# pavelacamposp/direct_data_driven_mpc

Measured on AMD Instinct MI355X. Metric: QP solves/sec (batched), four-tank robust DD-MPC L=30 N=400, higher is better.
Workload: dtype f64

## Files before the change

### direct_data_driven_mpc_amd/csrc/ddmpc_cold2.hpp

```cpp
#pragma once
#include "ddmpc_kernels.hpp"

namespace ddmpc {

template <int NT, int W>
struct TileMap2 {
  struct Tab { int wave[NT]; int base[NT]; int maxs; };
  static constexpr Tab make() {
    Tab t{};
    int load[W] = {};
    t.wave[0] = 0; t.base[0] = 0; load[0] = NT;
    for (int d = 1; d < NT; ++d) {
      int w = (W > 1) ? 1 : 0;
      for (int i = w + 1; i < W; ++i) if (load[i] < load[w]) w = i;
      t.wave[d] = w;
      t.base[d] = load[w];
      load[w] += NT - d;
    }
    t.maxs = 0;
    for (int i = 0; i < W; ++i) if (load[i] > t.maxs) t.maxs = load[i];
    return t;
  }
  static constexpr Tab tab = make();
  static constexpr int MAXS = tab.maxs;
  static constexpr int wave(int I, int J) { return tab.wave[I - J]; }
  static constexpr int slot(int I, int J) { return tab.base[I - J] + J; }
  static constexpr bool has_row(int w, int J) {
    for (int K = 0; K < J; ++K) if (wave(J, K) == w) return true;
    return false;
  }
  static constexpr bool has_col(int w, int J) {
    for (int I = J + 1; I < NT; ++I) if (wave(I, J) == w) return true;
    return false;
  }
};

template <int NT, int W, int WAVE>
struct WaveTiles2 {
  struct Tab { int I[NT * (NT + 1) / 2]; int J[NT * (NT + 1) / 2]; int n; };
  static constexpr Tab make() {
    Tab t{};
    t.n = 0;
    for (int J = 0; J < NT; ++J)
      for (int I = J; I < NT; ++I)
        if (TileMap2<NT, W>::wave(I, J) == WAVE) { t.I[t.n] = I; t.J[t.n] = J; ++t.n; }
    return t;
  }
  static constexpr Tab tab = make();
};

template <int CTRL>
__device__ __forceinline__ double dpp_mov_f64(double v) {
  const int lo = __builtin_amdgcn_update_dpp(0, __double2loint(v), CTRL, 0xf, 0xf, false);
  const int hi = __builtin_amdgcn_update_dpp(0, __double2hiint(v), CTRL, 0xf, 0xf, false);
  return __hiloint2double(hi, lo);
}
__device__ __forceinline__ double row16_total(double v) {
  v += dpp_mov_f64<0x128>(v);
  v += dpp_mov_f64<0x124>(v);
  v += dpp_mov_f64<0x122>(v);
  v += dpp_mov_f64<0x121>(v);
  return v;
}

__device__ __forceinline__ d2 permlane16_swap_f64(double a, double b) {
  const auto lo = __builtin_amdgcn_permlane16_swap((unsigned)__double2loint(a), (unsigned)__double2loint(b), false, false);
  const auto hi = __builtin_amdgcn_permlane16_swap((unsigned)__double2hiint(a), (unsigned)__double2hiint(b), false, false);
  return d2{__hiloint2double((int)hi[0], (int)lo[0]), __hiloint2double((int)hi[1], (int)lo[1])};
}

__device__ __forceinline__ double rsq_n2(double x) {
  const double y0 = __builtin_amdgcn_rsq(x);
  const double e = fma(-x * y0, y0, 1.0);
  return fma(0.5 * y0, e, y0);
}

__device__ __forceinline__ double rows4_total(double v) {
  const d2 s1 = permlane16_swap_f64(v, v);
  v = s1[0] + s1[1];
  const auto lo2 = __builtin_amdgcn_permlane32_swap((unsigned)__double2loint(v), (unsigned)__double2loint(v), false, false);
  const auto hi2 = __builtin_amdgcn_permlane32_swap((unsigned)__double2hiint(v), (unsigned)__double2hiint(v), false, false);
  return __hiloint2double((int)hi2[0], (int)lo2[0]) + __hiloint2double((int)hi2[1], (int)lo2[1]);
}

__device__ __forceinline__ double wave_max(double v) {
  v = fmax(v, dpp_mov_f64<0x128>(v));
  v = fmax(v, dpp_mov_f64<0x124>(v));
  v = fmax(v, dpp_mov_f64<0x122>(v));
  v = fmax(v, dpp_mov_f64<0x121>(v));
  const d2 s1 = permlane16_swap_f64(v, v);
  v = fmax(s1[0], s1[1]);
  const auto lo2 = __builtin_amdgcn_permlane32_swap((unsigned)__double2loint(v), (unsigned)__double2loint(v), false, false);
  const auto hi2 = __builtin_amdgcn_permlane32_swap((unsigned)__double2hiint(v), (unsigned)__double2hiint(v), false, false);
  return fmax(__hiloint2double((int)hi2[0], (int)lo2[0]), __hiloint2double((int)hi2[1], (int)lo2[1]));
}

template <int NT, int W>
struct Lds2 {
  static constexpr int RP = 16 * NT;
  static constexpr int dvec = 0;
  static constexpr int tvec = dvec + RP;
  static constexpr int beta = tvec + RP;
  static constexpr int cd0 = beta + RP;
  static constexpr int cd1 = cd0 + RP;
  static constexpr int ct0 = cd1 + RP;
  static constexpr int ckk = ct0 + RP;
  static constexpr int PART_LEN = 2 * 16 * W;
  static constexpr int part = ckk + (RP + 1) / 2;
  static constexpr int RED_LEN = 34;
  static constexpr int red = part + PART_LEN;
  static constexpr int ints = red + RED_LEN;
  static constexpr int INTS_LEN = (RP + 8 + 1) / 2;
  static constexpr int pt2 = (ints + INTS_LEN + 2) & ~1;
  static constexpr int PT2_LEN = 32 * 4;
  static constexpr int LRS = 36;
  static constexpr int lt16 = pt2 + PT2_LEN;
  static constexpr int LT_LEN = 16 * LRS;
  static constexpr int pastw = lt16;
  static constexpr int PASTW_CAP = LT_LEN / 2;
  static constexpr int cpp = lt16 + PASTW_CAP;
  static constexpr int RSB = RP + 4;
  static constexpr int pb = lt16 + LT_LEN;
  static constexpr int PB_LEN = 16 * RSB;
  static constexpr int ctab = pb + PB_LEN;
  static constexpr int CTAB_LEN = 4 * RP;
  static constexpr bool DST_ALIAS = RP >= 128;
  static constexpr int dst = ctab + CTAB_LEN;
  static constexpr int DST_LEN = (W > 1 && !DST_ALIAS) ? 256 : 0;
  static constexpr int dst_lo = DST_ALIAS ? dvec : dst;
  static constexpr int dst_hi = DST_ALIAS ? beta : dst + 128;
  static constexpr int xs = dst + DST_LEN;
  static constexpr int SCR = pt2;
  static constexpr int SCR_LEN = dst - pt2;
  __host__ __device__ static constexpr int total(int xs_len) { return (xs + xs_len + 1) & ~1; }

  static_assert(W >= 1 && W <= 8, "red[] keeps 8 per-wave slots per quantity; part[] is sized by W");
  static_assert(24 + W <= 32 && RED_LEN >= 33, "red[24 + w] and red[32] (output stage) must stay inside red[]");
  static_assert(pt2 >= ints + INTS_LEN && (pt2 & 1) == 0, "act[RP] + flags[8] end before the in-tile panel; 16-byte aligned");
  static_assert(cpp + (RP + 1) / 2 <= lt16 + LT_LEN, "prologue staging (past window + its index table) must fit inside lt16");
  static_assert(NT * 256 <= PB_LEN, "back substitution keeps the NT inverse diagonal tiles M_J in the panel buffer");
  static_assert(16 * (RP / 4) <= CTAB_LEN, "one 4x4 lag block per time step of the window");
  static_assert((xs & 1) == 0 && (lt16 & 1) == 0 && (pb & 1) == 0, "16-byte alignment of the regions accessed with b128");
};

template <int NT, int W>
struct Lds2Limits {
  static constexpr int max_past = Lds2<NT, W>::PASTW_CAP;
  static constexpr int scratch = Lds2<NT, W>::SCR_LEN;
};

template <int NT, int W, int WAVE, bool REF, bool CVX>
__device__ __forceinline__ void wave_body2(const KParams& P, double* __restrict__ sm,
                                           const double* __restrict__ up, const double* __restrict__ yp,
                                           double* __restrict__ u_opt, double* __restrict__ cost_out,
                                           int* __restrict__ status_out, int* __restrict__ iters_out,
                                           double* __restrict__ beta_ws, signed char* __restrict__ act_ws,
                                           unsigned long long* __restrict__ stamps, double* __restrict__ lfac,
                                           double* __restrict__ lfacT, int* __restrict__ refine_flag,
                                           int* __restrict__ refine_count, const double* __restrict__ gpre,
                                           const double* __restrict__ ud_b, const double* __restrict__ yd_b) {
  using TM = TileMap2<NT, W>;
  using WT = WaveTiles2<NT, W, WAVE>;
  using LD = Lds2<NT, W>;
  constexpr int RP = 16 * NT;
  constexpr int NTHR = 64 * W;
  constexpr int LRS = LD::LRS, RSB = LD::RSB;
  int nstamp = 1;
  auto stamp = [&]() __attribute__((always_inline)) {
    if (stamps != nullptr && WAVE == 0) {
      const unsigned long long t = __builtin_amdgcn_s_memtime();
      if (threadIdx.x == 0 && nstamp < 7) stamps[nstamp] = t;
      ++nstamp;
    }
  };
  double* xs = sm + LD::xs;
  double* dvec = sm + LD::dvec;
  double* tvec = sm + LD::tvec;
  double* beta = sm + LD::beta;
  double* part = sm + LD::part;
  double* red = sm + LD::red;
  double* ctab = sm + LD::ctab;
  double* PT2 = sm + LD::pt2;
  double* LT = sm + LD::lt16;
  double* PB = sm + LD::pb;
  int* act = reinterpret_cast<int*>(sm + LD::ints);
  int* flags = act + RP;

  int tid0 = threadIdx.x;
  asm volatile("" : "+v"(tid0));
  const int r = P.r, rE = P.rE, nch = P.nch;
  const int NS = rE >> 2;
  const int IR = rE >> 4;
  const int rr = rE & 15;

  constexpr int NHELP = (W > 1) ? W - 1 : 1;
  constexpr int DFIRST = 3;
  constexpr int NDSLOT = (W > 1 && NT > DFIRST) ? (NT - DFIRST + NHELP - 1) / NHELP : 1;
  auto downer = [](int J) constexpr { return 1 + (J - DFIRST) % NHELP; };
  auto dslot = [](int J) constexpr { return (J - DFIRST) / NHELP; };
  static_assert(8 * (TM::MAXS + (W > 1 ? NDSLOT : 0)) + 40 <= 512 / DDMPC_MIN_WAVES(NT, W),
                "the accumulator tiles of the busiest wave must leave a working set of 40 VGPRs at the occupancy of __launch_bounds__");
  d4 acc[TM::MAXS];
  d4 dlt[NDSLOT];
  double* DSTlo = sm + LD::dst_lo;
  double* DSThi = sm + LD::dst_hi;

  constexpr int NE = (RP + NTHR - 1) / NTHR;
  double* cD0 = sm + LD::cd0;
  double* cD1 = sm + LD::cd1;
  double* cT = sm + LD::ct0;
  int* cK = reinterpret_cast<int*>(sm + LD::ckk);
  {
    const int* cP = reinterpret_cast<const int*>(sm + LD::cpp);
    const double* pastw = sm + LD::pastw;
    static_for<NE>([&](auto e) __attribute__((always_inline)) {
      const int rho = tid0 + e * NTHR;
      if (rho < RP) {
        const int pidx = cP[rho];
        if (pidx >= 0) cT[rho] = pastw[pidx];
        act[rho] = 0;
      }
    });
  }
  if (tid0 < 8) flags[tid0] = 0;

  int iter = 0;
  int status = 0;
  int nupd = 0;
  bool ctab_ok = false;
  int tid = tid0;
  double kmax = 0.0;
  long long tphF = 0, tphB = 0, tphT = 0, tphA = 0, tphU = 0;
  const bool timing = (stamps != nullptr) && (WAVE == 0);
  auto now = [&]() __attribute__((always_inline)) -> long long { return timing ? (long long)__builtin_amdgcn_s_memtime() : 0; };
  for (;;) {
    ++iter;
    asm volatile("" : "+v"(tid));
    int r_it = P.r, rE_it = P.rE;
    asm volatile("" : "+s"(r_it), "+s"(rE_it));
    const int r = r_it, rE = rE_it;
    const int NS = rE >> 2, IR = rE >> 4, rr = rE & 15;
    const int lane = tid & 63;
    const int l15 = lane & 15, l4 = lane >> 4, l3 = lane & 3, lo = l15 >> 2;
    int ix_x = lane & 31, ix_lt = l4 * LRS + l15, ix_pw = l4 * 4 + l3;
    if constexpr (WAVE == 0) asm volatile("" : "+v"(ix_x), "+v"(ix_lt), "+v"(ix_pw));
    static_for<NE>([&](auto e) __attribute__((always_inline)) {
      const int rho = tid + e * NTHR;
      if (rho < RP) {
        const int s_act = act[rho];
        dvec[rho] = s_act ? cD1[rho] : cD0[rho];
        tvec[rho] = cT[rho] + s_act * P.bound;
        beta[rho] = 0.0;
      }
    });
    if (tid == 0) flags[1] = 0;
    __syncthreads();
    stamp();

    bool f0_done = false;
    static_for<NDSLOT>([&](auto S) __attribute__((always_inline)) { dlt[S] = d4{0.0, 0.0, 0.0, 0.0}; });
    bool dst_valid = false;
    auto fix_tile = [&](auto II, auto JJ, const d4& raw, const double dd) __attribute__((always_inline)) -> d4 {
      constexpr int I = II, J = JJ;
      const int gc = 16 * I + l15;
      d4 v = -raw;
      if constexpr (I == J) {
        const bool live = gc < r;
        const int dj = l15 - l4;
        static_for<4>([&](auto j) __attribute__((always_inline)) {
          const bool hit = live && (dj == 4 * j);
          if (hit) { asm volatile(""); kmax = fmax(kmax, raw[j()]); v[j()] -= P.lam * dd; }
        });
      }
      if (16 * I + 15 >= r) {
        double tg[4];
        static_for<4>([&](auto j) __attribute__((always_inline)) { tg[j()] = tvec[16 * J + l4 + 4 * j]; });
        double tc = 0.0;
        if constexpr (I == J) tc = tvec[gc];
        static_for<4>([&](auto j) __attribute__((always_inline)) {
          const int gr = 16 * J + l4 + 4 * j;
          if (gr >= r || gc >= r) v[j()] = 0.0;
          if (I == J && gr == gc && gr >= r && gr < rE) v[j()] = -1.0;
          if (gc == rE && gr < r) v[j()] = -tg[j()];
          if (I == J && gr == rE && gc < r) v[j()] = -tc;
        });
      }
      if (P.dense_w) {
        const double* dm = P.dmat + (long long)(16 * J + l4) * RP + 16 * I + l15;
        static_for<4>([&](auto j) __attribute__((always_inline)) { v[j()] -= P.lam * dm[4 * j() * RP]; });
      }
      return v;
    };
    auto substep = [&](d4& Ad, d4& Et, d4& Mt, auto QQ, auto&& pend) __attribute__((always_inline)) {
      constexpr int q = QQ;
      constexpr int c0 = 4 * q;
#define DDMPC_HOOK(h) do { pend(std::integral_constant<int, h>{}); } while (0)
      const double* Pr = PT2 + 4 * ix_x;
      const double* Pd = PT2 + c0 * 4;
      const double p00 = -Pd[0];
      const double p10 = -Pd[4], p11 = -Pd[5];
      const double p20 = -Pd[8], p21 = -Pd[9], p22 = -Pd[10];
      const double p30 = -Pd[12], p31 = -Pd[13], p32 = -Pd[14], p33 = -Pd[15];
      const double r0 = Pr[0], r1 = Pr[1], r2 = Pr[2], r3 = Pr[3];
      double m0 = 0.0, m1 = 0.0, m2 = 0.0;
      if constexpr (q == 3) {
        m0 = LT[ix_lt + 16]; m1 = LT[ix_lt + 4 * LRS + 16]; m2 = LT[ix_lt + 8 * LRS + 16];
      }
      DDMPC_HOOK(0);
      const double i0 = rsq_n2(p00);
      DDMPC_HOOK(1);
      const double l10 = p10 * i0, l20 = p20 * i0, l30 = p30 * i0;
      const double i1 = rsq_n2(p11 - l10 * l10);
      DDMPC_HOOK(2);
      const double l21 = (p21 - l20 * l10) * i1, l31 = (p31 - l30 * l10) * i1;
      const double i2 = rsq_n2(p22 - l20 * l20 - l21 * l21);
      DDMPC_HOOK(3);
      const double l32 = (p32 - l30 * l20 - l31 * l21) * i2;
      const double i3 = rsq_n2(p33 - l30 * l30 - l31 * l31 - l32 * l32);
      DDMPC_HOOK(4);
      const double x0 = -r0 * i0;
      const double x1 = -(r1 + x0 * l10) * i1;
      DDMPC_HOOK(5);
      const double x2 = -(r2 + x0 * l20 + x1 * l21) * i2;
      const double x3 = -(r3 + x0 * l30 + x1 * l31 + x2 * l32) * i3;
      DDMPC_HOOK(6);
      const d2 s01a = permlane16_swap_f64(x0, x1), s23a = permlane16_swap_f64(x2, x3);
      const bool lowhalf = lane < 32;
      const double opA = lowhalf ? s01a[0] : s23a[0];
      const double opE = lowhalf ? s01a[1] : s23a[1];
      LT[ix_lt + c0 * LRS] = opA;
      LT[ix_lt + c0 * LRS + 16] = opE;
      if constexpr (q == 3) Mt = d4{m0, m1, m2, opE};
      DDMPC_HOOK(7);
      if constexpr (q < 3) {
        Ad = __builtin_amdgcn_mfma_f64_16x16x4f64(opA, opA, Ad, 0, 0, 0);
        Et = __builtin_amdgcn_mfma_f64_16x16x4f64(opE, opA, Et, 0, 0, 0);
      }
      DDMPC_HOOK(8);
      DDMPC_HOOK(9);
      DDMPC_HOOK(10);
      DDMPC_HOOK(11);
      if constexpr (q < 3) {
        if (lo == q + 1) {
          static_for<4>([&](auto j) __attribute__((always_inline)) {
            PT2[ix_pw + 16 * j] = Ad[j()];
            PT2[ix_pw + 16 * j + 64] = Et[j()];
          });
        }
      }
      __builtin_amdgcn_fence(__ATOMIC_ACQ_REL, "wavefront");
#undef DDMPC_HOOK
    };
    auto no_pend = [](auto) __attribute__((always_inline)) {};
    auto factor_begin = [&](const d4& Ad, d4& Et) __attribute__((always_inline)) {
      int lz = lane;
      asm volatile("" : "+v"(lz));
      static_for<4>([&](auto j) __attribute__((always_inline)) { Et[j()] = ((lz >> 4) + 4 * j() == (lz & 15)) ? -1.0 : 0.0; });
      if (lo == 0) {
        static_for<4>([&](auto j) __attribute__((always_inline)) {
          PT2[ix_pw + 16 * j] = Ad[j()];
          PT2[ix_pw + 16 * j + 64] = Et[j()];
        });
      }
      __builtin_amdgcn_fence(__ATOMIC_ACQ_REL, "wavefront");
    };
    auto factor_end = [&](auto JT, int nq) __attribute__((always_inline)) {
      constexpr int Jt = JT;
      constexpr int SD = TM::slot(Jt, Jt);
      __builtin_amdgcn_fence(__ATOMIC_ACQ_REL, "wavefront");
      if (nq < 4) {
        static_for<4>([&](auto j) __attribute__((always_inline)) {
          const int k = l4 + 4 * j();
          const double mv = LT[k * LRS + 16 + l15];
          acc[SD][j()] = (k < 4 * nq) ? mv : 0.0;
        });
      }
      if (Jt == IR) {
        if (lane < 4 * nq) tvec[16 * Jt + lane] = LT[lane * LRS + rr];
      }
      if (lfac != nullptr) {
        static_for<4>([&](auto e) __attribute__((always_inline)) {
          const int idx = lane + 64 * e(), xr = idx >> 4, kc = idx & 15;
          double v = (kc <= xr && kc < 4 * nq) ? LT[kc * LRS + xr] : 0.0;
          if (xr == kc && kc >= 4 * nq) v = 1.0;
          lfac[(Jt * (Jt + 1) / 2 + Jt) * 256 + idx] = v;
          lfacT[(Jt * (Jt + 1) / 2 + Jt) * 256 + kc * 16 + xr] = v;
        });
      }
    };
    if (gpre != nullptr) {
      static_for<WT::tab.n>([&](auto K) __attribute__((always_inline)) {
        constexpr int I = WT::tab.I[K], J = WT::tab.J[K];
        acc[TM::slot(I, J)] = *reinterpret_cast<const d4*>(gpre + (I * (I + 1) / 2 + J) * 256 + 4 * lane);
      });
      stamp();
      stamp();
    } else if (P.gram_dense) {
      static_for<TM::MAXS>([&](auto S) __attribute__((always_inline)) { acc[S] = d4{0.0, 0.0, 0.0, 0.0}; });
      const int c = P.c;
      const int cfull = c & ~3;
      const double* xp = xs + l4 * nch + l15;
      for (int i0 = 0; i0 < cfull; i0 += 4) {
        double op[NT];
        static_for<NT>([&](auto I) __attribute__((always_inline)) { op[I] = xp[16 * I]; });
        xp += 4 * nch;
        static_for<WT::tab.n>([&](auto K) __attribute__((always_inline)) {
          constexpr int I = WT::tab.I[K], J = WT::tab.J[K];
          acc[TM::slot(I, J)] = __builtin_amdgcn_mfma_f64_16x16x4f64(op[J], op[I], acc[TM::slot(I, J)], 0, 0, 0);
        });
      }
      if (cfull < c) {
        const bool kok = (cfull + l4) < c;
        double op[NT];
        static_for<NT>([&](auto I) __attribute__((always_inline)) { const double v = xp[16 * I]; op[I] = kok ? v : 0.0; });
        static_for<WT::tab.n>([&](auto K) __attribute__((always_inline)) {
          constexpr int I = WT::tab.I[K], J = WT::tab.J[K];
          acc[TM::slot(I, J)] = __builtin_amdgcn_mfma_f64_16x16x4f64(op[J], op[I], acc[TM::slot(I, J)], 0, 0, 0);
        });
      }
      stamp();
      stamp();
    } else {
      const int nsub = (nch == 2) ? 2 : 1;
      const int Ln = (nch == 2) ? (P.Ln + 1) >> 1 : P.Ln;
      auto csub = [&](int sub) __attribute__((always_inline)) { return (nch == 2) ? ((P.c + 1 - sub) >> 1) : P.c; };
      {
        constexpr int TS = (W >= 4) ? 4 : W;
        constexpr int GS = W / TS;
        constexpr int MAXG = (NT + GS - 1) / GS;
        static_assert(TS * GS == W, "waves = time slices x group slices");
        static_assert(TS * GS * MAXG * 64 <= LD::PT2_LEN + LD::LT_LEN + LD::PB_LEN, "partial lag blocks fit between pt2 and ctab");
        const int ngroups = (Ln + 3) >> 2;
        const int kq = lane >> 4, blk = (lane >> 2) & 3, ij = lane & 3;
        double* PP = sm + LD::pt2;
        constexpr int tsl = WAVE % TS, gsl = WAVE / TS;
        const bool need_lag = CVX ? !ctab_ok : (iter == 1);
        if (need_lag) {
          double cacc[MAXG];
          static_for<MAXG>([&](auto gi) __attribute__((always_inline)) { cacc[gi()] = 0.0; });
#pragma nounroll
          for (int sub = 0; sub < nsub; ++sub) {
          const int c = csub(sub);
          const double* xb = xs + 2 * sub;
          const int cfull = c & ~3;
          const int nks = cfull >> 2;
          const int kw = (nks + TS - 1) / TS;
          const int ks0 = tsl * kw;
          const int ks1 = (ks0 + kw) < nks ? (ks0 + kw) : nks;
          const double* pB = xb + 4 * (kq + 4 * ks0) + ij;
          const double* pA = xb + 4 * (kq + blk + 4 * ks0) + ij + 16 * (gsl * MAXG);
          auto ld = [&](double (&bv)[4], double (&av)[MAXG + 3]) __attribute__((always_inline)) {
            static_for<4>([&](auto u) __attribute__((always_inline)) { bv[u()] = pB[16 * u]; });
            static_for<MAXG + 3>([&](auto q) __attribute__((always_inline)) { av[q()] = pA[16 * q]; });
            pA += 64; pB += 64;
          };
          auto mm = [&](const double (&bv)[4], const double (&av)[MAXG + 3]) __attribute__((always_inline)) {
            static_for<4>([&](auto u) __attribute__((always_inline)) {
              static_for<MAXG>([&](auto gi) __attribute__((always_inline)) {
                cacc[gi()] = __builtin_amdgcn_mfma_f64_4x4x4f64(av[gi() + u()], bv[u()], cacc[gi()], 0, 0, 0);
              });
            });
          };
          const int nk = ks1 > ks0 ? ks1 - ks0 : 0;
          const int ntrip = nk >> 2;
          double bv0[4], av0[MAXG + 3];
#pragma nounroll
          for (int it = 0; it < ntrip; ++it) {
            ld(bv0, av0);
            mm(bv0, av0);
          }
          for (int k = 4 * ntrip; k < nk; ++k) {
            const double bv = pB[0];
            static_for<MAXG>([&](auto gi) __attribute__((always_inline)) {
              cacc[gi()] = __builtin_amdgcn_mfma_f64_4x4x4f64(pA[16 * gi], bv, cacc[gi()], 0, 0, 0);
            });
            pA += 16; pB += 16;
          }
          if (tsl == TS - 1 && cfull < c) {
            const bool kok = (cfull + kq) < c;
            const double bv = kok ? pB[0] : 0.0;
            static_for<MAXG>([&](auto gi) __attribute__((always_inline)) {
              const double a1 = pA[16 * gi];
              cacc[gi()] = __builtin_amdgcn_mfma_f64_4x4x4f64(kok ? a1 : 0.0, bv, cacc[gi()], 0, 0, 0);
            });
          }
          }
          static_for<MAXG>([&](auto gi) __attribute__((always_inline)) {
            PP[((tsl * GS + gsl) * MAXG + gi()) * 64 + lane] = cacc[gi()];
          });
        }
        __syncthreads();
        if (need_lag) {
          for (int e = tid; e < GS * MAXG * 64; e += NTHR) {
            const int g = e >> 6, ln = e & 63;
            double sacc = 0.0;
            static_for<TS>([&](auto t) __attribute__((always_inline)) { sacc += PP[(t() * GS * MAXG + g) * 64 + ln]; });
            const int d = 4 * g + ((ln >> 2) & 3);
            if (g < ngroups && d < Ln) ctab[d * 16 + (ln >> 4) * 4 + (ln & 3)] = sacc;
          }
        }
      }
      __syncthreads();
      ctab_ok = true;
      stamp();
      static_for<TM::MAXS>([&](auto S) __attribute__((always_inline)) { acc[S] = d4{0.0, 0.0, 0.0, 0.0}; });
      {
#pragma nounroll
        for (int d = 0; d < NT; ++d) {
          bool mine = false;
          static_for<NT>([&](auto DD) __attribute__((always_inline)) {
            if constexpr (TM::tab.wave[DD] == WAVE) mine = mine || (d == DD);
          });
          if (!mine) continue;
          auto base = [&](int j) __attribute__((always_inline)) -> double {
            int del = 4 * d + lo - j;
            const bool neg = del < 0;
            del = neg ? -del : del;
            del = del >= Ln ? Ln - 1 : del;
            const int pa = neg ? l4 : l3, pb = neg ? l3 : l4;
            const int nl = neg ? lo : j;
            double t = ctab[del * 16 + pa * 4 + pb];
#pragma nounroll
            for (int sub = 0; sub < nsub; ++sub) {
              const int c = csub(sub);
              const double* qa0 = xs + 2 * sub + 4 * del + pa;
              const double* qa1 = qa0 + 4 * c;
              const double* qb0 = xs + 2 * sub + pb;
              const double* qb1 = qb0 + 4 * c;
              const double e0 = qa1[0] * qb1[0] - qa0[0] * qb0[0];
              const double e1 = qa1[4] * qb1[4] - qa0[4] * qb0[4];
              const double e2 = qa1[8] * qb1[8] - qa0[8] * qb0[8];
              t += (0 < nl) ? e0 : 0.0;
              t += (1 < nl) ? e1 : 0.0;
              t += (2 < nl) ? e2 : 0.0;
            }
            return t;
          };
          const d4 v = d4{base(0), base(1), base(2), base(3)};
          static_for<NT>([&](auto DD) __attribute__((always_inline)) {
            if constexpr (TM::tab.wave[DD] == WAVE) { if (d == DD) acc[TM::slot(DD, 0)] = v; }
          });
        }
      }
      static_for<NT>([&](auto DD) __attribute__((always_inline)) {
        constexpr int d = DD;
        if constexpr (TM::tab.wave[d] == WAVE && d + 1 < NT) {
          const double* pb = xs + 4 * l4 + l15;
          const double* pa = pb + 16 * d;
          auto walk = [&](auto NSUB) __attribute__((always_inline)) {
            constexpr bool two = NSUB() == 2;
            const double* pa2 = pa + 4 * csub(0);
            const double* pb2 = pb + 4 * csub(0);
            const double* pa4 = pa + 2 + 4 * csub(1);
            const double* pb4 = pb + 2 + 4 * csub(1);
            double n_a1 = pa[0], n_b1 = pb[0], n_a2 = pa2[0], n_b2 = pb2[0];
            double n_a3 = 0.0, n_b3 = 0.0, n_a4 = 0.0, n_b4 = 0.0;
            if constexpr (two) { n_a3 = pa[2]; n_b3 = pb[2]; n_a4 = pa4[0]; n_b4 = pb4[0]; }
            static_for<NT - d - 1>([&](auto T) __attribute__((always_inline)) {
              const double a1 = n_a1, b1 = n_b1, a2 = n_a2, b2 = n_b2, a3 = n_a3, b3 = n_b3, a4 = n_a4, b4 = n_b4;
              if constexpr (T() + 1 < NT - d - 1) {
                constexpr int o = 16 * (T() + 1);
                n_a1 = pa[o]; n_b1 = pb[o]; n_a2 = pa2[o]; n_b2 = pb2[o];
                if constexpr (two) { n_a3 = pa[o + 2]; n_b3 = pb[o + 2]; n_a4 = pa4[o]; n_b4 = pb4[o]; }
              }
              d4 v = __builtin_amdgcn_mfma_f64_16x16x4f64(-b1, a1, acc[TM::slot(d + T, T)], 0, 0, 0);
              if constexpr (two) {
                v = __builtin_amdgcn_mfma_f64_16x16x4f64(-b3, a3, v, 0, 0, 0);
                v = __builtin_amdgcn_mfma_f64_16x16x4f64(b4, a4, v, 0, 0, 0);
              }
              acc[TM::slot(d + T + 1, T + 1)] = __builtin_amdgcn_mfma_f64_16x16x4f64(b2, a2, v, 0, 0, 0);
            });
          };
          if (nsub == 2) walk(std::integral_constant<int, 2>{});
          else walk(std::integral_constant<int, 1>{});
        }
      });
      if constexpr (WAVE == 0 && W > 1) {
        if (rE >= 16) {
          constexpr int S0 = TM::slot(0, 0);
          d4 Ad = fix_tile(std::integral_constant<int, 0>{}, std::integral_constant<int, 0>{}, acc[S0], dvec[l15]);
          d4 Et;
          factor_begin(Ad, Et);
          static_for<4>([&](auto q) __attribute__((always_inline)) { substep(Ad, Et, acc[S0], q, no_pend); });
          factor_end(std::integral_constant<int, 0>{}, 4);
          f0_done = true;
        }
      }
      stamp();
    }

    const long long tfx0 = now();
    double dgv[NT];
    static_for<WT::tab.n>([&](auto K) __attribute__((always_inline)) {
      constexpr int I = WT::tab.I[K], J = WT::tab.J[K];
      if constexpr (I == J) dgv[J] = dvec[16 * J + l15];
    });
    static_for<WT::tab.n>([&](auto K) __attribute__((always_inline)) {
      constexpr int I = WT::tab.I[K], J = WT::tab.J[K];
      constexpr int S = TM::slot(I, J);
      if (!(I == 0 && J == 0 && f0_done))
        acc[S] = fix_tile(std::integral_constant<int, I>{}, std::integral_constant<int, J>{}, acc[S], I == J ? dgv[J] : 0.0);
    });
    const long long tfx1 = now();
    if constexpr (W > 1 && WAVE >= 1 && WAVE <= 3) {
      if (stamps != nullptr) {
        const unsigned long long th = __builtin_amdgcn_s_memtime();
        if (lane == 0) stamps[6 + WAVE] = th << 32;
      }
    }
    __syncthreads();
    if constexpr (!CVX) {
      if (timing && threadIdx.x == 0) {
        const long long tfx2 = now();
        stamps[10] = (unsigned long long)(tfx1 - tfx0) << 32;
        stamps[11] = (unsigned long long)(tfx2 - tfx1) << 32;
      }
    }

    {
      const int nq0 = NS < 4 ? NS : 4;
      const long long t0 = now();
      if constexpr (WAVE == 0) {
        if (!f0_done) {
          d4 Ad = acc[TM::slot(0, 0)];
          d4 Et;
          factor_begin(Ad, Et);
          static_for<4>([&](auto q) __attribute__((always_inline)) { if (q() < nq0) substep(Ad, Et, acc[TM::slot(0, 0)], q, no_pend); });
          factor_end(std::integral_constant<int, 0>{}, nq0);
        }
      }
      const long long t1 = now();
      __syncthreads();
      tphF += t1 - t0; tphB += now() - t1;
    }
    static_for<NT>([&](auto JB) __attribute__((always_inline)) {
      constexpr int Jb = JB;
      const int nqc = (NS - 4 * Jb) < 4 ? (NS - 4 * Jb) : 4;
      if (nqc > 0) {
        const bool more = 16 * (Jb + 1) < rE + 1;
        const int nqn = (NS - 4 * (Jb + 1)) < 4 ? (NS - 4 * (Jb + 1)) : 4;
        const long long t0 = now();
        if constexpr (WAVE == 0 && W > 1 && Jb >= 1 && Jb + DFIRST - 1 < NT) {
          if (dst_valid) {
            constexpr int SDn = TM::slot(Jb + DFIRST - 1, Jb + DFIRST - 1);
            acc[SDn][0] += DSTlo[lane]; acc[SDn][1] += DSTlo[64 + lane];
            acc[SDn][2] += DSThi[lane]; acc[SDn][3] += DSThi[64 + lane];
          }
        }
        dst_valid = false;
        double am[4];
        static_for<4>([&](auto ks) __attribute__((always_inline)) { am[ks()] = -LT[l15 * LRS + 16 + 4 * ks() + l4]; });
        auto trsm_tile = [&](auto II) __attribute__((always_inline)) {
          constexpr int I = II;
          if (16 * I < rE + 1) {
            constexpr int S = TM::slot(I, Jb);
            const d4 T = acc[S];
            d4 dd = d4{0.0, 0.0, 0.0, 0.0};
            dd = __builtin_amdgcn_mfma_f64_16x16x4f64(am[0], T[0], dd, 0, 0, 0);
            dd = __builtin_amdgcn_mfma_f64_16x16x4f64(am[1], T[1], dd, 0, 0, 0);
            dd = __builtin_amdgcn_mfma_f64_16x16x4f64(am[2], T[2], dd, 0, 0, 0);
            dd = __builtin_amdgcn_mfma_f64_16x16x4f64(am[3], T[3], dd, 0, 0, 0);
            acc[S] = dd;
            static_for<4>([&](auto j) __attribute__((always_inline)) { PB[(l4 + 4 * j) * RSB + 16 * I + l15] = dd[j()]; });
          }
        };
        if constexpr (Jb + 1 < NT) {
          if constexpr (TM::wave(Jb + 1, Jb) == WAVE) { if (more) trsm_tile(std::integral_constant<int, Jb + 1>{}); }
        }
        const long long t1 = now();
        __syncthreads();
        const long long t2 = now();
        d4 Ad = d4{0.0, 0.0, 0.0, 0.0}, Et = d4{0.0, 0.0, 0.0, 0.0};
        if constexpr (WAVE == 0 && Jb + 1 < NT) {
          if (nqn > 0) {
            constexpr int S = TM::slot(Jb + 1, Jb + 1);
            Ad = acc[S];
            const long long tu0 = now();
            static_for<4>([&](auto ks) __attribute__((always_inline)) {
              const double o = PB[(4 * ks() + l4) * RSB + 16 * (Jb + 1) + l15];
              Ad = __builtin_amdgcn_mfma_f64_16x16x4f64(o, o, Ad, 0, 0, 0);
            });
            tphU += now() - tu0;
            factor_begin(Ad, Et);
            substep(Ad, Et, acc[S], std::integral_constant<int, 0>{}, no_pend);
          }
        }
        if (more) {
          static_for<NT>([&](auto I) __attribute__((always_inline)) {
            if constexpr (I > Jb + 1 && TM::wave(I, Jb) == WAVE) trsm_tile(I);
          });
        }
        const long long t3 = now();
        __syncthreads();
        const long long t4 = now();
        if constexpr (WAVE == 0 && Jb + 1 < NT) {
          static_for<3>([&](auto QM) __attribute__((always_inline)) {
            constexpr int q = QM + 1;
            constexpr int first = Jb + 2 + QM;
            constexpr int last = (W > 1) ? ((Jb + DFIRST - 1 < NT - 1) ? Jb + DFIRST - 1 : NT - 1) : NT - 1;
            constexpr int ntl = first <= last ? (last - first) / 3 + 1 : 0;
            auto pend = [&](auto H) __attribute__((always_inline)) {
              constexpr int h0 = H;
              static_for<(4 * ntl + 11) / 12>([&](auto R) __attribute__((always_inline)) {
                constexpr int h = h0 + 12 * R;
                if constexpr (h < 4 * ntl) {
                  constexpr int J2 = first + 3 * (h % ntl), ks = h / ntl;
                  constexpr int S2 = TM::slot(J2, J2);
                  const double o = PB[(4 * ks + l4) * RSB + 16 * J2 + l15];
                  acc[S2] = __builtin_amdgcn_mfma_f64_16x16x4f64(o, o, acc[S2], 0, 0, 0);
                }
              });
            };
            if (q < nqn) substep(Ad, Et, acc[TM::slot(Jb + 1, Jb + 1)], std::integral_constant<int, q>{}, pend);
          });
          if (nqn > 0) factor_end(std::integral_constant<int, Jb + 1>{}, nqn);
        }
        if (more) {
          static_for<4>([&](auto ks) __attribute__((always_inline)) {
            double op[NT];
            static_for<NT>([&](auto X) __attribute__((always_inline)) {
              if constexpr (X > Jb) op[X] = PB[(4 * ks() + l4) * RSB + 16 * X + l15];
            });
            static_for<WT::tab.n>([&](auto K) __attribute__((always_inline)) {
              constexpr int I = WT::tab.I[K], J = WT::tab.J[K];
              if constexpr (J > Jb && I > J) {
                if (16 * I < rE + 1) {
                  constexpr int S = TM::slot(I, J);
                  acc[S] = __builtin_amdgcn_mfma_f64_16x16x4f64(op[J], op[I], acc[S], 0, 0, 0);
                }
              }
            });
            if constexpr (WAVE != 0 && W > 1) {
              static_for<NT>([&](auto JD) __attribute__((always_inline)) {
                constexpr int J = JD;
                if constexpr (J >= Jb + DFIRST) {
                  if constexpr (downer(J) == WAVE) {
                    if (16 * J < rE + 1) dlt[dslot(J)] = __builtin_amdgcn_mfma_f64_16x16x4f64(op[J], op[J], dlt[dslot(J)], 0, 0, 0);
                  }
                }
              });
            }
          });
          if constexpr (W > 1 && Jb + DFIRST < NT) {
            if constexpr (WAVE != 0) {
              if constexpr (downer(Jb + DFIRST) == WAVE) {
                const d4 dv = dlt[dslot(Jb + DFIRST)];
                DSTlo[lane] = dv[0]; DSTlo[64 + lane] = dv[1]; DSThi[lane] = dv[2]; DSThi[64 + lane] = dv[3];
              }
            }
            dst_valid = true;
          }
        }
        const long long t5 = now();
        __syncthreads();
        const long long t6 = now();
        tphT += t1 - t0; tphA += (t2 - t1) + (t4 - t3); tphF += (t3 - t2) + (t5 - t4); tphB += t6 - t5;
      }
    });
    if (timing && threadIdx.x == 0) {
      constexpr unsigned long long HI = 0xffffffff00000000ull;
      stamps[7] = (stamps[7] & HI) | (unsigned long long)tphF; stamps[8] = (stamps[8] & HI) | (unsigned long long)tphB;
      if constexpr (CVX) { stamps[9] &= HI; stamps[10] = 0; stamps[11] = 0; }
      else { stamps[9] = (stamps[9] & HI) | (unsigned long long)tphT; stamps[10] += tphA; stamps[11] += tphU; }
    }
    stamp();

    if (lfac != nullptr) {
      static_for<WT::tab.n>([&](auto K) __attribute__((always_inline)) {
        constexpr int I = WT::tab.I[K], J = WT::tab.J[K];
        if constexpr (I > J) {
          constexpr int S = TM::slot(I, J);
          static_for<4>([&](auto j) __attribute__((always_inline)) {
            lfacT[(I * (I + 1) / 2 + J) * 256 + (l4 + 4 * j) * 16 + l15] = acc[S][j()];
            lfac[(I * (I + 1) / 2 + J) * 256 + l15 * 16 + l4 + 4 * j] = acc[S][j()];
          });
        }
      });
    }

    static_for<WT::tab.n>([&](auto K) __attribute__((always_inline)) {
      constexpr int I = WT::tab.I[K], J = WT::tab.J[K];
      if constexpr (I > J) {
        if (I == IR && l15 == rr) {
          constexpr int S = TM::slot(I, J);
          static_for<4>([&](auto j) __attribute__((always_inline)) { tvec[16 * J + l4 + 4 * j] = acc[S][j()]; });
        }
      }
    });
    auto back_substitute = [&](double* __restrict__ out, const double* __restrict__ yin, const int rE) __attribute__((always_inline)) {
      double* Mb = PB;
      constexpr int CW = TM::wave(1, 0);
      auto far_col = [](int w, int J) constexpr { for (int I = J + 2; I < NT; ++I) if (TM::wave(I, J) == w) return true; return false; };
      if constexpr (WAVE == 0) {
        static_for<NT>([&](auto J) __attribute__((always_inline)) {
          if (16 * J < rE) {
            constexpr int SD = TM::slot(J, J);
            static_for<4>([&](auto j) __attribute__((always_inline)) { Mb[J * 256 + (l4 + 4 * j) * 16 + l15] = acc[SD][j()]; });
          }
        });
      }
      __syncthreads();
      double xl[NT];
      static_for<NT>([&](auto I) __attribute__((always_inline)) { xl[I] = 0.0; });
      d4 Ct = d4{0.0, 0.0, 0.0, 0.0};
      d4 xk = d4{0.0, 0.0, 0.0, 0.0};
      static_for<NT>([&](auto JREV) __attribute__((always_inline)) {
        constexpr int J = NT - 1 - JREV;
        if (16 * J < rE) {
          if constexpr (WAVE == CW) {
            const double* pr = part + (J & 1) * (16 * W);
            double pi = 0.0;
            static_for<4>([&](auto j) __attribute__((always_inline)) {
              const int k = l4 + 4 * j();
              double v = yin[16 * J + k];
              if constexpr (J + 2 < NT) {
                if (16 * (J + 2) < rE) {
                  static_for<W>([&](auto w) __attribute__((always_inline)) {
                    if constexpr (far_col(w(), J)) v -= pr[w * 16 + k];
                  });
                }
              }
              pi = fma(Mb[J * 256 + k * 16 + l15], v, pi);
            });
            static_for<4>([&](auto q) __attribute__((always_inline)) { pi = fma(-Ct[q()], xk[q()], pi); });
            pi = rows4_total(pi);
            xl[J] = (16 * J + l15 < rE) ? pi : 0.0;
            if (l4 == 0) out[16 * J + l15] = xl[J];
            if constexpr (J >= 1) {
              constexpr int S = TM::slot(J, J - 1);
              Ct = d4{0.0, 0.0, 0.0, 0.0};
              static_for<4>([&](auto j) __attribute__((always_inline)) {
                Ct = __builtin_amdgcn_mfma_f64_16x16x4f64(acc[S][j()], Mb[(J - 1) * 256 + (4 * j() + l4) * 16 + l15], Ct, 0, 0, 0);
              });
              __builtin_amdgcn_fence(__ATOMIC_ACQ_REL, "wavefront");
              static_for<4>([&](auto q) __attribute__((always_inline)) { xk[q()] = out[16 * J + l4 + 4 * q()]; });
            }
          }
          if constexpr (J >= 1) {
            if constexpr (far_col(WAVE, J - 1)) {
              if (16 * (J + 1) < rE) {
                d4 sv = d4{0.0, 0.0, 0.0, 0.0};
                static_for<NT>([&](auto I) __attribute__((always_inline)) {
                  if constexpr (I >= J + 1 && TM::wave(I, J - 1) == WAVE) {
                    constexpr int S = TM::slot(I, J - 1);
                    static_for<4>([&](auto j) __attribute__((always_inline)) { sv[j()] = fma(acc[S][j()], xl[I], sv[j()]); });
                  }
                });
                static_for<4>([&](auto j) __attribute__((always_inline)) { sv[j()] = row16_total(sv[j()]); });
                if (l15 == 0) {
                  double* pw = part + ((J - 1) & 1) * (16 * W);
                  static_for<4>([&](auto j) __attribute__((always_inline)) { pw[WAVE * 16 + l4 + 4 * j] = sv[j()]; });
                }
              }
            }
          }
          __syncthreads();
          if constexpr (WAVE != CW) xl[J] = out[16 * J + l15];
        }
      });
    };
    auto forward_substitute = [&]() __attribute__((always_inline)) {
      static_for<NT>([&](auto JJ) __attribute__((always_inline)) {
        constexpr int J = JJ;
        if (16 * J < rE) {
          if constexpr (TM::has_row(WAVE, J)) {
            double s = 0.0;
            static_for<J>([&](auto K) __attribute__((always_inline)) {
              if constexpr (TM::wave(J, K) == WAVE) {
                constexpr int S = TM::slot(J, K);
                static_for<4>([&](auto j) __attribute__((always_inline)) {
                  s = fma(acc[S][j()], tvec[16 * K + l4 + 4 * j()], s);
                });
              }
            });
            s = rows4_total(s);
            if (l4 == 0) part[WAVE * 16 + l15] = s;
          }
          __syncthreads();
          if constexpr (WAVE == 0) {
            constexpr int SD = TM::slot(J, J);
            double v = tvec[16 * J + l15];
            static_for<W>([&](auto w) __attribute__((always_inline)) {
              if constexpr (TM::has_row(w, J)) v -= part[w * 16 + l15];
            });
            v = (16 * J + l15 < rE) ? v : 0.0;
            d4 q;
            static_for<4>([&](auto j) __attribute__((always_inline)) { q[j()] = row16_total(acc[SD][j()] * v); });
            if (l15 == 0) {
              static_for<4>([&](auto j) __attribute__((always_inline)) { tvec[16 * J + l4 + 4 * j] = q[j()]; });
            }
          }
          __syncthreads();
        }
      });
    };
    back_substitute(beta, tvec, rE);

    if constexpr (REF) {
    if (P.refine != 0 && P.lam != 0.0) {
      bool go = true;
      double prev = 1e300;
      for (int pass = 0; go && pass < P.refine_max; ++pass) {
        const int c = P.c;
        constexpr int CHF = 16 * RSB;
        const bool windowed = P.stage_xs == 0;
// ... 660 lines not shown
```

Baseline: 14.20 million.

## Fold Gram negation into MFMA signs and split tile fixup into diag/pad/dense passes

Negation of the Gram tiles moves into the accumulation itself: MFMA operand signs are flipped, and the precomputed and dense paths negate on load. The monolithic fix_tile is split into fix_diag, fix_pad and fix_dense, with the pad and dense fixes applied only to tiles that need them. The lag base-tile computation is unrolled per sub-channel count with loads hoisted ahead of use. The aim is to cut per-tile fixup VALU work and branches before factorization. It moves diagonal fixing onto wave 0 for all diagonal slots, which relies on the slot-to-wave mapping, and changes where stamps are taken.

```diff
diff --git a/direct_data_driven_mpc_amd/csrc/ddmpc_cold2.hpp b/direct_data_driven_mpc_amd/csrc/ddmpc_cold2.hpp
--- a/direct_data_driven_mpc_amd/csrc/ddmpc_cold2.hpp
+++ b/direct_data_driven_mpc_amd/csrc/ddmpc_cold2.hpp
@@ -260,36 +260,38 @@
     bool f0_done = false;
     static_for<NDSLOT>([&](auto S) __attribute__((always_inline)) { dlt[S] = d4{0.0, 0.0, 0.0, 0.0}; });
     bool dst_valid = false;
-    auto fix_tile = [&](auto II, auto JJ, const d4& raw, const double dd) __attribute__((always_inline)) -> d4 {
+    auto fix_diag = [&](auto JJ, d4& v, const double dd) __attribute__((always_inline)) {
+      constexpr int J = JJ;
+      const bool live = 16 * J + l15 < r;
+      const int dj = live ? l15 - l4 : -1;
+      double e[4] = {v[0], v[1], v[2], v[3]};
+      static_for<4>([&](auto j) __attribute__((always_inline)) {
+        int dq = dj;
+        asm volatile("" : "+v"(dq));
+        const bool hit = dq == 4 * j;
+        if (hit) { asm volatile(""); kmax = fmax(kmax, -e[j()]); e[j()] = fma(-P.lam, dd, e[j()]); }
+      });
+      v = d4{e[0], e[1], e[2], e[3]};
+    };
+    auto fix_pad = [&](auto II, auto JJ, d4& v) __attribute__((always_inline)) {
       constexpr int I = II, J = JJ;
       const int gc = 16 * I + l15;
-      d4 v = -raw;
-      if constexpr (I == J) {
-        const bool live = gc < r;
-        const int dj = l15 - l4;
-        static_for<4>([&](auto j) __attribute__((always_inline)) {
-          const bool hit = live && (dj == 4 * j);
-          if (hit) { asm volatile(""); kmax = fmax(kmax, raw[j()]); v[j()] -= P.lam * dd; }
-        });
-      }
-      if (16 * I + 15 >= r) {
-        double tg[4];
-        static_for<4>([&](auto j) __attribute__((always_inline)) { tg[j()] = tvec[16 * J + l4 + 4 * j]; });
-        double tc = 0.0;
-        if constexpr (I == J) tc = tvec[gc];
-        static_for<4>([&](auto j) __attribute__((always_inline)) {
-          const int gr = 16 * J + l4 + 4 * j;
-          if (gr >= r || gc >= r) v[j()] = 0.0;
-          if (I == J && gr == gc && gr >= r && gr < rE) v[j()] = -1.0;
-          if (gc == rE && gr < r) v[j()] = -tg[j()];
-          if (I == J && gr == rE && gc < r) v[j()] = -tc;
-        });
-      }
-      if (P.dense_w) {
-        const double* dm = P.dmat + (long long)(16 * J + l4) * RP + 16 * I + l15;
-        static_for<4>([&](auto j) __attribute__((always_inline)) { v[j()] -= P.lam * dm[4 * j() * RP]; });
-      }
-      return v;
+      double tg[4];
+      static_for<4>([&](auto j) __attribute__((always_inline)) { tg[j()] = tvec[16 * J + l4 + 4 * j]; });
+      double tc = 0.0;
+      if constexpr (I == J) tc = tvec[gc];
+      static_for<4>([&](auto j) __attribute__((always_inline)) {
+        const int gr = 16 * J + l4 + 4 * j;
+        if (gr >= r || gc >= r) v[j()] = 0.0;
+        if (I == J && gr == gc && gr >= r && gr < rE) v[j()] = -1.0;
+        if (gc == rE && gr < r) v[j()] = -tg[j()];
+        if (I == J && gr == rE && gc < r) v[j()] = -tc;
+      });
+    };
+    auto fix_dense = [&](auto II, auto JJ, d4& v) __attribute__((always_inline)) {
+      constexpr int I = II, J = JJ;
+      const double* dm = P.dmat + (long long)(16 * J + l4) * RP + 16 * I + l15;
+      static_for<4>([&](auto j) __attribute__((always_inline)) { v[j()] = fma(-P.lam, dm[4 * j() * RP], v[j()]); });
     };
     auto substep = [&](d4& Ad, d4& Et, d4& Mt, auto QQ, auto&& pend) __attribute__((always_inline)) {
       constexpr int q = QQ;
@@ -388,14 +390,14 @@
         });
       }
     };
+    const bool structured = gpre == nullptr && !P.gram_dense;
     if (gpre != nullptr) {
       static_for<WT::tab.n>([&](auto K) __attribute__((always_inline)) {
         constexpr int I = WT::tab.I[K], J = WT::tab.J[K];
-        acc[TM::slot(I, J)] = *reinterpret_cast<const d4*>(gpre + (I * (I + 1) / 2 + J) * 256 + 4 * lane);
+        acc[TM::slot(I, J)] = -*reinterpret_cast<const d4*>(gpre + (I * (I + 1) / 2 + J) * 256 + 4 * lane);
       });
       stamp();
-      stamp();
-    } else if (P.gram_dense) {
+    } else if (!structured) {
       static_for<TM::MAXS>([&](auto S) __attribute__((always_inline)) { acc[S] = d4{0.0, 0.0, 0.0, 0.0}; });
       const int c = P.c;
       const int cfull = c & ~3;
@@ -418,7 +420,10 @@
           acc[TM::slot(I, J)] = __builtin_amdgcn_mfma_f64_16x16x4f64(op[J], op[I], acc[TM::slot(I, J)], 0, 0, 0);
         });
       }
-      stamp();
+      static_for<WT::tab.n>([&](auto K) __attribute__((always_inline)) {
+        constexpr int S = TM::slot(WT::tab.I[K], WT::tab.J[K]);
+        acc[S] = -acc[S];
+      });
       stamp();
     } else {
       const int nsub = (nch == 2) ? 2 : 1;
@@ -505,6 +510,40 @@
       stamp();
       static_for<TM::MAXS>([&](auto S) __attribute__((always_inline)) { acc[S] = d4{0.0, 0.0, 0.0, 0.0}; });
       {
+        auto base_tile = [&](const int d, auto NSUB) __attribute__((always_inline)) -> d4 {
+          constexpr int nsb = NSUB();
+          auto base = [&](int j) __attribute__((always_inline)) -> double {
+            int del = 4 * d + lo - j;
+            const bool neg = del < 0;
+            del = neg ? -del : del;
+            del = del >= Ln ? Ln - 1 : del;
+            const int pa = neg ? l4 : l3, pb = neg ? l3 : l4;
+            const int nl = neg ? lo : j;
+            double va0[nsb][3], va1[nsb][3], vb0[nsb][3], vb1[nsb][3];
+            double t = ctab[del * 16 + pa * 4 + pb];
+            static_for<nsb>([&](auto sub) __attribute__((always_inline)) {
+              const int c = csub(sub());
+              const double* qa0 = xs + 2 * sub() + 4 * del + pa;
+              const double* qa1 = qa0 + 4 * c;
+              const double* qb0 = xs + 2 * sub() + pb;
+              const double* qb1 = qb0 + 4 * c;
+              static_for<3>([&](auto k) __attribute__((always_inline)) {
+                va0[sub()][k()] = qa0[4 * k()]; va1[sub()][k()] = qa1[4 * k()];
+                vb0[sub()][k()] = qb0[4 * k()]; vb1[sub()][k()] = qb1[4 * k()];
+              });
+            });
+            static_for<nsb>([&](auto sub) __attribute__((always_inline)) {
+              const double e0 = va1[sub()][0] * vb1[sub()][0] - va0[sub()][0] * vb0[sub()][0];
+              const double e1 = va1[sub()][1] * vb1[sub()][1] - va0[sub()][1] * vb0[sub()][1];
+              const double e2 = va1[sub()][2] * vb1[sub()][2] - va0[sub()][2] * vb0[sub()][2];
+              t += (0 < nl) ? e0 : 0.0;
+              t += (1 < nl) ? e1 : 0.0;
+              t += (2 < nl) ? e2 : 0.0;
+            });
+            return t;
+          };
+          return d4{base(0), base(1), base(2), base(3)};
+        };
 #pragma nounroll
         for (int d = 0; d < NT; ++d) {
           bool mine = false;
@@ -512,31 +551,10 @@
             if constexpr (TM::tab.wave[DD] == WAVE) mine = mine || (d == DD);
           });
           if (!mine) continue;
-          auto base = [&](int j) __attribute__((always_inline)) -> double {
-            int del = 4 * d + lo - j;
-            const bool neg = del < 0;
-            del = neg ? -del : del;
-            del = del >= Ln ? Ln - 1 : del;
-            const int pa = neg ? l4 : l3, pb = neg ? l3 : l4;
-            const int nl = neg ? lo : j;
-            double t = ctab[del * 16 + pa * 4 + pb];
-#pragma nounroll
-            for (int sub = 0; sub < nsub; ++sub) {
-              const int c = csub(sub);
-              const double* qa0 = xs + 2 * sub + 4 * del + pa;
-              const double* qa1 = qa0 + 4 * c;
-              const double* qb0 = xs + 2 * sub + pb;
-              const double* qb1 = qb0 + 4 * c;
-              const double e0 = qa1[0] * qb1[0] - qa0[0] * qb0[0];
-              const double e1 = qa1[4] * qb1[4] - qa0[4] * qb0[4];
-              const double e2 = qa1[8] * qb1[8] - qa0[8] * qb0[8];
-              t += (0 < nl) ? e0 : 0.0;
-              t += (1 < nl) ? e1 : 0.0;
-              t += (2 < nl) ? e2 : 0.0;
-            }
-            return t;
-          };
-          const d4 v = d4{base(0), base(1), base(2), base(3)};
+          d4 v;
+          if (nsub == 2) v = base_tile(d, std::integral_constant<int, 2>{});
+          else v = base_tile(d, std::integral_constant<int, 1>{});
+          v = -v;
           static_for<NT>([&](auto DD) __attribute__((always_inline)) {
             if constexpr (TM::tab.wave[DD] == WAVE) { if (d == DD) acc[TM::slot(DD, 0)] = v; }
           });
@@ -563,22 +581,29 @@
                 n_a1 = pa[o]; n_b1 = pb[o]; n_a2 = pa2[o]; n_b2 = pb2[o];
                 if constexpr (two) { n_a3 = pa[o + 2]; n_b3 = pb[o + 2]; n_a4 = pa4[o]; n_b4 = pb4[o]; }
               }
-              d4 v = __builtin_amdgcn_mfma_f64_16x16x4f64(-b1, a1, acc[TM::slot(d + T, T)], 0, 0, 0);
+              d4 v = __builtin_amdgcn_mfma_f64_16x16x4f64(b1, a1, acc[TM::slot(d + T, T)], 0, 0, 0);
               if constexpr (two) {
-                v = __builtin_amdgcn_mfma_f64_16x16x4f64(-b3, a3, v, 0, 0, 0);
-                v = __builtin_amdgcn_mfma_f64_16x16x4f64(b4, a4, v, 0, 0, 0);
+                v = __builtin_amdgcn_mfma_f64_16x16x4f64(b3, a3, v, 0, 0, 0);
+                v = __builtin_amdgcn_mfma_f64_16x16x4f64(-b4, a4, v, 0, 0, 0);
               }
-              acc[TM::slot(d + T + 1, T + 1)] = __builtin_amdgcn_mfma_f64_16x16x4f64(b2, a2, v, 0, 0, 0);
+              acc[TM::slot(d + T + 1, T + 1)] = __builtin_amdgcn_mfma_f64_16x16x4f64(-b2, a2, v, 0, 0, 0);
             });
           };
           if (nsub == 2) walk(std::integral_constant<int, 2>{});
           else walk(std::integral_constant<int, 1>{});
         }
       });
-      if constexpr (WAVE == 0 && W > 1) {
-        if (rE >= 16) {
-          constexpr int S0 = TM::slot(0, 0);
-          d4 Ad = fix_tile(std::integral_constant<int, 0>{}, std::integral_constant<int, 0>{}, acc[S0], dvec[l15]);
+    }
+    if constexpr (WAVE == 0) {
+      constexpr int S0 = TM::slot(0, 0);
+      double dgw[NT];
+      static_for<NT>([&](auto J) __attribute__((always_inline)) { dgw[J] = dvec[16 * J + l15]; });
+      static_for<NT>([&](auto J) __attribute__((always_inline)) { fix_diag(J, acc[TM::slot(J, J)], dgw[J()]); });
+      if (15 >= r) fix_pad(std::integral_constant<int, 0>{}, std::integral_constant<int, 0>{}, acc[S0]);
+      if (P.dense_w) fix_dense(std::integral_constant<int, 0>{}, std::integral_constant<int, 0>{}, acc[S0]);
+      if constexpr (W > 1) {
+        if (structured && rE >= 16) {
+          d4 Ad = acc[S0];
           d4 Et;
           factor_begin(Ad, Et);
           static_for<4>([&](auto q) __attribute__((always_inline)) { substep(Ad, Et, acc[S0], q, no_pend); });
@@ -586,21 +611,30 @@
           f0_done = true;
         }
       }
-      stamp();
-    }
+    }
+    stamp();
 
     const long long tfx0 = now();
-    double dgv[NT];
     static_for<WT::tab.n>([&](auto K) __attribute__((always_inline)) {
       constexpr int I = WT::tab.I[K], J = WT::tab.J[K];
-      if constexpr (I == J) dgv[J] = dvec[16 * J + l15];
+      if constexpr (I == NT - 1) {
+        if (16 * I + 15 >= r) fix_pad(std::integral_constant<int, I>{}, std::integral_constant<int, J>{}, acc[TM::slot(I, J)]);
+      }
     });
-    static_for<WT::tab.n>([&](auto K) __attribute__((always_inline)) {
-      constexpr int I = WT::tab.I[K], J = WT::tab.J[K];
-      constexpr int S = TM::slot(I, J);
-      if (!(I == 0 && J == 0 && f0_done))
-        acc[S] = fix_tile(std::integral_constant<int, I>{}, std::integral_constant<int, J>{}, acc[S], I == J ? dgv[J] : 0.0);
-    });
+    if (16 * (NT - 2) + 15 >= r) {
+      static_for<WT::tab.n>([&](auto K) __attribute__((always_inline)) {
+        constexpr int I = WT::tab.I[K], J = WT::tab.J[K];
+        if constexpr (I < NT - 1 && I > 0) {
+          if (16 * I + 15 >= r) fix_pad(std::integral_constant<int, I>{}, std::integral_constant<int, J>{}, acc[TM::slot(I, J)]);
+        }
+      });
+    }
+    if (P.dense_w) {
+      static_for<WT::tab.n>([&](auto K) __attribute__((always_inline)) {
+        constexpr int I = WT::tab.I[K], J = WT::tab.J[K];
+        if constexpr (I > 0) fix_dense(std::integral_constant<int, I>{}, std::integral_constant<int, J>{}, acc[TM::slot(I, J)]);
+      });
+    }
     const long long tfx1 = now();
     if constexpr (W > 1 && WAVE >= 1 && WAVE <= 3) {
       if (stamps != nullptr) {
```

Result: no change. 14.18 million (-0.2%).
